# zprihoda/zopt

Hardware: AMD Instinct MI355X
Metric: LQR horizon-steps/sec (batch x T) at n=12,m=4,T=50 (higher is better)
Workload: dtype f64; 1 GPU; discreteFiniteHorizonLqr: 4096 random LTI systems per GPU, n=12 m=4 T=50 fp64, A/B/Q/R materialised (b,T,.,.), BASELINE configs[1]; batch_per_gpu=4096, T=50, n=12, m=4, parallelism=batch-sharded x1

## Files before the change

### zopt_amd/csrc/ilqr_backward.hip

```cpp
#include "dma_ring.h"
#include "models.h"
#include "ns16.h"
#include "tile16_f64.h"
#include "zm_common.h"

#include <cstdlib>

namespace zm {

template <int KS>
struct IlqrStepRegs {
    double F[KS];
    double C[KS];
    double Cu;
    double cv;
    double dc;
    double dr[KS];
};

struct TrajList {
    const int* list;
    long count;
};

template <int KS>
struct IlqrAddr {
    const double* pF0;
    const double* pC0;
    const double* pCu;
    const double* pcv;
    const double* pdc;
    const double* pdr0;
    const double* pz[4];
    int sz[4], stz[4];
    int zc[4];
    bool zlive[4];
    double* pOut;
    int dF, dC, sF, sC, sCu, scv, sOut, sd;
    bool rowok[KS], vF[KS], vC[KS], vCu, vcv, vOut, vL, cA;
    double vsum = 0.0;
    double cu_pad;
};

template <int KS, int MODE>
__device__ __forceinline__ void ilqr_load_step(IlqrStepRegs<KS>& d, IlqrAddr<KS>& a) {
    double f[KS], cc[KS];
#pragma unroll
    for (int s = 0; s < KS; ++s) f[s] = a.pF0[a.rowok[s] ? s * a.dF : 0];
    a.pF0 -= a.sF;
#pragma unroll
    for (int s = 0; s < KS; ++s) cc[s] = a.pC0[a.rowok[s] ? s * a.dC : 0];
    a.pC0 -= a.sC;
    const double cu = *a.pCu;
    a.pCu -= a.sCu;
    const double cv = *a.pcv;
    a.pcv -= a.scv;
#pragma unroll
    for (int s = 0; s < KS; ++s) {
        d.F[s] = a.vF[s] ? f[s] : 0.0;
        d.C[s] = a.vC[s] ? cc[s] : 0.0;
    }
    d.Cu = a.vCu ? cu : a.cu_pad;
    d.cv = a.vcv ? cv : 0.0;
    if constexpr (MODE == 1) {
        const double dc = *a.pdc;
        double dr[KS];
#pragma unroll
        for (int s = 0; s < KS; ++s) dr[s] = a.pdr0[a.rowok[s] ? 4 * s : 0];
        a.pdc -= a.sd;
        a.pdr0 -= a.sd;
        d.dc = a.cA ? dc : 0.0;
#pragma unroll
        for (int s = 0; s < KS; ++s) d.dr[s] = a.rowok[s] ? dr[s] : 0.0;
    }
}

constexpr int ILQR_LDS_DOUBLES = 116;

#ifdef ZM_SWEEP_LAB
__device__ unsigned long long zm_sweep_stamps[10];
struct SweepLab {
    unsigned long long acc[8], last;
};
#define ZM_SWEEP_STAMP(lab, q)                                                                         \
    do {                                                                                              \
        unsigned long long t_;                                                                        \
        asm volatile("s_memtime %0\n\ts_waitcnt lgkmcnt(0)" : "=s"(t_)::"memory");                    \
        (lab)->acc[q] += t_ - (lab)->last;                                                            \
        (lab)->last = t_;                                                                             \
    } while (0)
#else
struct SweepLab {};
#define ZM_SWEEP_STAMP(lab, q) do { } while (0)
#endif

__device__ __forceinline__ void ilqr_lds_sync() { wave_lds_sync(); }

template <int KS, int MODE, bool PREFETCH, bool ZIN = false>
__device__ __forceinline__ void ilqr_step(double (&Vxx)[KS], double (&vxr)[KS], IlqrStepRegs<KS>& d, IlqrAddr<KS>& a,
                                          double* sm, const int g, const int c, const int ob0, const int ob1,
                                          const int ob2, const int ob3, const int oqa, double* jA, const int n,
                                          const int m, const d4 zin = d4{0.0, 0.0, 0.0, 0.0}, SweepLab* lab = nullptr) {
    constexpr int NP = 4 * KS;
    d4 pz = zero4();
    if constexpr (MODE == 2 && ZIN) {
        d4 zt = zin;
        psd_project_ns<KS + 1, true>(zt, a.zlive, 1e-3, jA, g, c);
        pz = zt;
    } else if constexpr (MODE == 2) {
        double z[4] = {0.0, 0.0, 0.0, 0.0};
#pragma unroll
        for (int i0 = 0; i0 < NP; i0 += 4) {
            double fz[4][4];
#pragma unroll
            for (int i = 0; i < 4; ++i) {
                const int ic = (i0 + i) < n ? (i0 + i) : 0;
#pragma unroll
                for (int r = 0; r < 4; ++r) fz[i][r] = a.pz[r][(long)ic * a.sz[r]];
            }
#pragma unroll
            for (int i = 0; i < 4; ++i) {
                const double vxi = (i0 + i) < n ? sm[80 + i0 + i] : 0.0;
#pragma unroll
                for (int r = 0; r < 4; ++r) z[r] = __builtin_fma(vxi, fz[i][r], z[r]);
            }
        }
        d4 zt;
#pragma unroll
        for (int r = 0; r < 4; ++r) {
            a.pz[r] -= a.stz[r];
            zt[r] = (a.zc[r] >= 0) ? z[r] : 0.0;
        }
        psd_project_ns<KS + 1>(zt, a.zlive, 1e-3, jA, g, c);
        pz = zt;
    }
    d4 y = zero4();
#pragma unroll
    for (int s = 0; s < KS; ++s) y = mfma(Vxx[s], d.F[s], y);
    d4 gacc = zero4();
#pragma unroll
    for (int s = 0; s < KS; ++s) gacc[s] = d.C[s] + pz[s];
    gacc[KS] = d.Cu + pz[KS];
#pragma unroll
    for (int s = 0; s < KS; ++s) gacc = mfma(y[s], d.F[s], gacc);
    double qp = 0.0;
    if constexpr (MODE == 1) {
        double vtd = 0.0;
#pragma unroll
        for (int s = 0; s < KS; ++s) vtd = __builtin_fma(Vxx[s], d.dr[s], vtd);
        vtd = sum_xor16(vtd);
        vtd = sum_xor32(vtd);
        if (g == 0) sm[96 + c] = a.cA ? vtd : 0.0;
        ilqr_lds_sync();
#pragma unroll
        for (int s = 0; s < KS; ++s) {
            double vd = Vxx[s] * d.dc;
            vd = row16_sum(vd);
            const double w = vxr[s] + (a.cA ? vd : sm[96 + 4 * s + g]);
            qp = __builtin_fma(d.F[s], w, qp);
        }
    } else {
#pragma unroll
        for (int s = 0; s < KS; ++s) qp = __builtin_fma(d.F[s], vxr[s], qp);
    }
    qp = sum_xor16(qp);
    qp = sum_xor32(qp);
    const double qv = d.cv + qp;
    if constexpr (PREFETCH) ilqr_load_step<KS, MODE>(d, a);

    ZM_SWEEP_STAMP(lab, 2);
    sm[g * 16 + c] = gacc[KS];
    if (g == 0) sm[64 + c] = qv;
    __builtin_amdgcn_fence(__ATOMIC_RELEASE, "wavefront");
    __builtin_amdgcn_wave_barrier();
    __builtin_amdgcn_fence(__ATOMIC_ACQUIRE, "wavefront");
    double S[4][4], b[4], x[4];
#pragma unroll
    for (int i = 0; i < 4; ++i) {
#pragma unroll
        for (int jj = 0; jj < 4; ++jj) S[i][jj] = sm[i * 16 + NP + jj];
    }
    b[0] = sm[ob0];
    b[1] = sm[ob1];
    b[2] = sm[ob2];
    b[3] = sm[ob3];
    const double quu_a = sm[oqa];
    __builtin_amdgcn_wave_barrier();
    const double b0[4] = {b[0], b[1], b[2], b[3]};
    ZM_SWEEP_STAMP(lab, 3);
    if (__builtin_amdgcn_ballot_w64(!lu_solve4_nopivot(S, b, x)) != 0ull) lu_solve4_fallback(S, b, x);
    {
        double keep = x[0] + x[1] + x[2] + x[3];
        asm volatile("" : "+v"(keep));
    }
    ZM_SWEEP_STAMP(lab, 4);
    const double x01 = (g & 1) ? x[1] : x[0];
    const double x23 = (g & 1) ? x[3] : x[2];
    const double xg = (g & 2) ? x23 : x01;
    const double out = (MODE == 1) ? xg : -xg;
    if (a.vOut) *a.pOut = out;
    a.pOut -= a.sOut;
    const double lv = a.vL ? out : 0.0;
    double qu[4];
    if constexpr (MODE != 1) {
#pragma unroll
        for (int i = 0; i < 4; ++i) qu[i] = sm[64 + NP + i];
    }
    if constexpr (MODE != 1) {
        if (c == NP) a.vsum -= 0.5 * ((x[0] * qu[0] + x[1] * qu[1]) + (x[2] * qu[2] + x[3] * qu[3]));
    }

    double vxn = qv;
    if constexpr (MODE == 1) {
        if (g == 0 && c == NP) {
#pragma unroll
            for (int i = 0; i < 4; ++i) sm[112 + i] = x[i];
        }
        ilqr_lds_sync();
#pragma unroll
        for (int i = 0; i < 4; ++i) vxn = __builtin_fma(-b0[i], sm[112 + i], vxn);
    } else {
#pragma unroll
        for (int i = 0; i < 4; ++i) vxn = __builtin_fma(-x[i], qu[i], vxn);
    }
    if (g == 0) sm[80 + c] = a.cA ? vxn : 0.0;
    const d4 t1 = mfma(quu_a, lv, zero4());
    d4 vacc = zero4();
#pragma unroll
    for (int s = 0; s < KS; ++s) vacc[s] = gacc[s];
    vacc = mfma<true>(lv, t1[0], vacc);
#pragma unroll
    for (int s = 0; s < KS; ++s) Vxx[s] = vacc[s];
    ilqr_lds_sync();
#pragma unroll
    for (int s = 0; s < KS; ++s) vxr[s] = sm[80 + 4 * s + g];
    __builtin_amdgcn_wave_barrier();
    ZM_SWEEP_STAMP(lab, 5);
}

template <int KS, int MODE>
__global__ __launch_bounds__(64, 2) void ilqr_backward_t16_f64(
    const double* __restrict__ f_x, const double* __restrict__ f_u, const double* __restrict__ c_x,
    const double* __restrict__ c_u, const double* __restrict__ c_xx, const double* __restrict__ c_ux,
    const double* __restrict__ c_uu, const double* __restrict__ vf_x, const double* __restrict__ vf_xx,
    const double* __restrict__ dvec, const double* __restrict__ f_xx, const double* __restrict__ f_ux,
    const double* __restrict__ f_uu, const long svx, const long svxx, const int* __restrict__ active,
    const int shared_h, double* __restrict__ lout, double* __restrict__ Lout, const int T, const int n, const int m,
    const double* __restrict__ c_s, const double* __restrict__ vf_s, double* __restrict__ v_out,
    double* __restrict__ vx_out, double* __restrict__ vxx_out, const TrajList tl, const double* __restrict__ Hpk,
    const PairTab ptab) {
    constexpr int NP = 4 * KS;
    const int lane = threadIdx.x;
    const long traj = tl.list ? (long)tl.list[blockIdx.x] : (long)blockIdx.x;
    if (active && active[traj] == 0) return;
    const int g = lane >> 4, c = lane & 15;
    __shared__ double sm[ILQR_LDS_DOUBLES];
    __shared__ double jA[MODE == 2 ? NS_LDS_DOUBLES : 1];

    IlqrAddr<KS> a;
    const int nn = n * n, nm = n * m, mm = m * m;
    const bool cA = c < n;
    a.cA = cA;
    const bool cB = (c >= NP) && (c < NP + m);
    const long last = traj * T + (T - 1);
    const double* fxt = f_x + last * nn;
    const double* fut = f_u + last * nm;
    const double* cxt = c_x + last * n;
    const double* cut = c_u + last * m;
    const double* cxxt = shared_h ? c_xx : c_xx + last * nn;
    const double* cuxt = shared_h ? c_ux : c_ux + last * nm;
    const double* cuut = shared_h ? c_uu : c_uu + last * mm;
    a.sC = shared_h ? 0 : nn;
    const bool row0 = g < n;
    const bool laneA = row0 && cA, laneB = row0 && cB;
    a.dF = laneA ? 4 * n : laneB ? 4 * m : 0;
    a.sF = laneB ? nm : nn;
    a.dC = laneA ? 4 * n : 0;
#pragma unroll
    for (int s = 0; s < KS; ++s) {
        const int row = 4 * s + g;
        a.rowok[s] = row < n;
        a.vF[s] = (row < n) && (cA || cB);
        a.vC[s] = (row < n) && cA;
    }
    a.pF0 = laneA ? (fxt + g * n + c) : laneB ? (fut + g * m + (c - NP)) : fxt;
    a.pC0 = laneA ? (cxxt + g * n + c) : cxxt;
    const bool vux = (g < m) && cA, vuu = (g < m) && cB;
    a.vCu = vux || vuu;
    a.pCu = vux ? (cuxt + g * n + c) : vuu ? (cuut + g * m + (c - NP)) : cuxt;
    a.sCu = shared_h ? 0 : (vuu ? mm : nm);
    a.cu_pad = (g >= m && c == NP + g) ? 1.0 : 0.0;
    a.vcv = cA || cB;
    a.pcv = cA ? (cxt + c) : cB ? (cut + (c - NP)) : cxt;
    a.scv = cB ? m : n;
    if constexpr (MODE == 1) {
        const double* dt_ = dvec + last * n;
        a.pdc = cA ? (dt_ + c) : dt_;
        a.pdr0 = row0 ? (dt_ + g) : dt_;
        a.sd = n;
    }
    if constexpr (MODE == 2) {
        const long nnn = (long)nn * n, nmn = (long)nm * n, nmm = (long)nm * m;
        const double* fxxt = f_xx + last * nnn;
        const double* fuxt = f_ux + last * nmn;
        const double* fuut = f_uu + last * nmm;
#pragma unroll
        for (int r = 0; r < 4; ++r) {
            const int row = 4 * r + g;
            const bool rx = row < n, ru = (row >= NP) && (row < NP + m);
            const int ca = rx ? row : (ru ? n + (row - NP) : -1);
            const int cb = cA ? c : (cB ? n + (c - NP) : -1);
            a.zc[r] = (ca >= 0 && cb >= 0) ? ca * 17 + cb : -1;
            a.zlive[r] = (ca >= 0) && (row == c);
            if (Hpk != nullptr) {
                int pidx = -1;
                if (ca >= 0 && cb >= 0) {
                    const int lo = ca < cb ? ca : cb, hi = ca < cb ? cb : ca;
                    for (int q = 0; q < ptab.n; ++q) pidx = (ptab.ab[q] == (unsigned char)(lo * 16 + hi)) ? q : pidx;
                }
                const double* Hl = Hpk + last * (long)ptab.n * n;
                if (pidx >= 0) {
                    a.pz[r] = Hl + (long)pidx * n;  a.sz[r] = 1;  a.stz[r] = ptab.n * n;
                } else {
                    a.pz[r] = Hl;  a.sz[r] = 0;  a.stz[r] = ptab.n * n;
                    a.zc[r] = -1;
                }
            } else if (f_ux == nullptr && !(rx && cA)) {
                a.zc[r] = -1;
                a.pz[r] = fxxt;  a.sz[r] = 0;  a.stz[r] = (int)nnn;
            } else if (rx && cA) {
                a.pz[r] = fxxt + row * n + c;  a.sz[r] = nn;  a.stz[r] = (int)nnn;
            } else if (rx && cB) {
                a.pz[r] = fuxt + (c - NP) * n + row;  a.sz[r] = nm;  a.stz[r] = (int)nmn;
            } else if (ru && cA) {
                a.pz[r] = fuxt + (row - NP) * n + c;  a.sz[r] = nm;  a.stz[r] = (int)nmn;
            } else if (ru && cB) {
                a.pz[r] = fuut + (row - NP) * m + (c - NP);  a.sz[r] = mm;  a.stz[r] = (int)nmm;
            } else {
                a.pz[r] = fxxt;  a.sz[r] = 0;  a.stz[r] = (int)nnn;
            }
        }
    }
    a.vL = (g < m) && cA;
    const bool vl = (g < m) && (c == NP);
    a.vOut = a.vL || vl;
    a.pOut = a.vL ? (Lout + last * nm + g * n + c) : (lout + last * m + g);
    a.sOut = vl ? m : nm;

    const bool rhs_qu = (c == NP);
    const int ob0 = rhs_qu ? (64 + NP + 0) : (0 * 16 + c);
    const int ob1 = rhs_qu ? (64 + NP + 1) : (1 * 16 + c);
    const int ob2 = rhs_qu ? (64 + NP + 2) : (2 * 16 + c);
    const int ob3 = rhs_qu ? (64 + NP + 3) : (3 * 16 + c);
    const int oqa = (c < 4) ? (c * 16 + NP + g) : (g * 16 + c);

    double Vxx[KS], vxr[KS];
    {
        const double* vxx = shared_h ? vf_xx : vf_xx + traj * svxx;
        const double* vx = vf_x + traj * svx;
#pragma unroll
        for (int s = 0; s < KS; ++s) {
            const int row = 4 * s + g;
            const bool ok = (row < n) && cA;
            const double t = vxx[ok ? row * n + c : 0];
            Vxx[s] = ok ? t : 0.0;
            const double u = vx[row < n ? row : 0];
            vxr[s] = (row < n) ? u : 0.0;
        }
    }

    if (g == 0) sm[80 + c] = cA ? (vf_x + traj * svx)[c] : 0.0;
    ilqr_lds_sync();
    if constexpr (MODE == 2) {
        for (int k2 = T - 1; k2 >= 0; --k2) {
            IlqrStepRegs<KS> d;
            ilqr_load_step<KS, MODE>(d, a);
            ilqr_step<KS, MODE, false>(Vxx, vxr, d, a, sm, g, c, ob0, ob1, ob2, ob3, oqa, jA, n, m);
        }
    } else {
    IlqrStepRegs<KS> d0, d1;
    ilqr_load_step<KS, MODE>(d0, a);
    if (T >= 2) ilqr_load_step<KS, MODE>(d1, a);
    int k = T - 1;
    while (k >= 3) {
        ilqr_step<KS, MODE, true>(Vxx, vxr, d0, a, sm, g, c, ob0, ob1, ob2, ob3, oqa, jA, n, m);
        ilqr_step<KS, MODE, true>(Vxx, vxr, d1, a, sm, g, c, ob0, ob1, ob2, ob3, oqa, jA, n, m);
        k -= 2;
    }
    if (k == 2) {
        ilqr_step<KS, MODE, true>(Vxx, vxr, d0, a, sm, g, c, ob0, ob1, ob2, ob3, oqa, jA, n, m);
        ilqr_step<KS, MODE, false>(Vxx, vxr, d1, a, sm, g, c, ob0, ob1, ob2, ob3, oqa, jA, n, m);
        ilqr_step<KS, MODE, false>(Vxx, vxr, d0, a, sm, g, c, ob0, ob1, ob2, ob3, oqa, jA, n, m);
    } else if (k == 1) {
        ilqr_step<KS, MODE, false>(Vxx, vxr, d0, a, sm, g, c, ob0, ob1, ob2, ob3, oqa, jA, n, m);
        ilqr_step<KS, MODE, false>(Vxx, vxr, d1, a, sm, g, c, ob0, ob1, ob2, ob3, oqa, jA, n, m);
    } else {
        ilqr_step<KS, MODE, false>(Vxx, vxr, d0, a, sm, g, c, ob0, ob1, ob2, ob3, oqa, jA, n, m);
    }
    }
    if (vxx_out) {
#pragma unroll
        for (int s = 0; s < KS; ++s) {
            const int row = 4 * s + g;
            if (row < n && cA) vxx_out[traj * nn + row * n + c] = Vxx[s];
        }
    }
    if (vx_out && g == 0 && cA) vx_out[traj * n + c] = sm[80 + c];
    if (v_out) {
        double cs = 0.0;
        if (c_s)
            for (int k2 = lane; k2 < T; k2 += 64) cs += c_s[traj * T + k2];
#pragma unroll
        for (int off = 32; off >= 1; off >>= 1) cs += __shfl_xor(cs, off, 64);
        if (g == 0 && c == NP) v_out[traj] = ((vf_s ? vf_s[traj] : 0.0) + cs) + a.vsum;
    }
}

}


namespace zm {

struct JacTab {
    unsigned char pos[12 * 16];
};
struct HTab {
    unsigned short dense[96];
    int n;
};
template <int N, int M, bool SHARED, int MODE, int NPAIR = 0, int NJP = 0, int NHS = 0>
struct IlqrDmaGeom {
    static constexpr int KS = N / 4;
    static constexpr int CFX = NJP ? NJP / 2 : N * N / 2, CFU = NJP ? 0 : N * M / 2, CCX = N / 2, CCU = M / 2;
    static constexpr int CXX = SHARED ? 0 : N * N / 2, CUX = SHARED ? 0 : N * M / 2, CUU = SHARED ? 0 : M * M / 2;
    static constexpr int CD = (MODE == 1) ? N / 2 : 0;
    static constexpr int CH = (MODE == 2) ? (NHS ? NHS / 2 : NPAIR * N / 2) : 0;
    static constexpr int CT = CFX + CFU + CCX + CCU + CXX + CUX + CUU + CD + CH;
    static constexpr int NI = (CT + 63) / 64;
    static constexpr int SLOT = NI * 1024;
    static constexpr int OFX = 0, OFU = CFX * 16, OCX = OFU + CFU * 16, OCU = OCX + CCX * 16;
    static constexpr int OXX = OCU + CCU * 16, OUX = OXX + CXX * 16, OUU = OUX + CUX * 16;
    static constexpr int OD = OUU + CUU * 16;
    static constexpr int OH = OD + CD * 16;
    static constexpr int OZ = CT * 16;
    static constexpr int OONE = OZ + 16;
    static_assert(NJP % 2 == 0 && (NJP == 0 || (N == 12 && SHARED)), "packed Jacobians: n = 12, 16-B rows, shared cost Hessians");
    static_assert(NJP == 0 || SLOT - OZ >= 32, "slot needs a zero and a one chunk");
    static_assert(N % 4 == 0 && N >= 8 && N <= 12 && M == 4, "fast path: all K-step rows live, m = 4");
    static_assert(MODE == 0 || (MODE == 1 && !SHARED) || (MODE == 2 && SHARED && N == 12 && NPAIR > 0 && NPAIR <= ZM_MAX_PAIRS),
                  "iLQR, affine LQR, or DDP with shared cost Hessians and packed second derivatives");
    static_assert(SLOT - OZ >= 16, "slot needs zero padding");
};

constexpr int ILQR_DMA_WAVES = 3, DDP_DMA_WAVES = 2;
template <int N, int M, int D, bool SHARED, int MODE, int NPAIR = 0, int NJP = 0, int NHS = 0, int W = 1>
__global__ __launch_bounds__(64 * W, MODE == 2 ? DDP_DMA_WAVES : ILQR_DMA_WAVES) void ilqr_backward_dma_f64(
    const double* __restrict__ f_x, const double* __restrict__ f_u, const double* __restrict__ c_x,
    const double* __restrict__ c_u, const double* __restrict__ c_xx, const double* __restrict__ c_ux,
    const double* __restrict__ c_uu, const double* __restrict__ vf_x, const double* __restrict__ vf_xx,
    const double* __restrict__ dvec, const long svx, const long svxx, const int* __restrict__ active,
    double* __restrict__ lout, double* __restrict__ Lout, const int T, const TrajList tl, const double* __restrict__ Hpk,
    const PairTab ptab, const JacTab jtab, const HTab htab) {
    using G = IlqrDmaGeom<N, M, SHARED, MODE, NPAIR, NJP, NHS>;
    static_assert(NHS % 2 == 0 && NHS <= 96 && (NHS == 0 || MODE == 2), "sparse second derivatives: DDP mode, 16-B rows");
    constexpr int KS = G::KS, NI = G::NI, SLOT = G::SLOT, NP = N;
    constexpr int nn = N * N, nm = N * M, mm = M * M;
    constexpr int SMO = D * SLOT;
    constexpr int HDN = NHS ? NPAIR * N : 0;
    constexpr int PER_WAVE = SMO + ILQR_LDS_DOUBLES * 8 + (MODE == 2 ? NS_LDS_DOUBLES * 8 : 0) + HDN * 8;
    static_assert(PER_WAVE % 16 == 0, "per-wave LDS slices stay 16-B aligned");
    __shared__ __attribute__((aligned(16))) char lds_all[W * PER_WAVE];
    const int wave = (W == 1) ? 0 : __builtin_amdgcn_readfirstlane((int)(threadIdx.x >> 6));
    char* const lds = lds_all + wave * PER_WAVE;
    double* sm = (double*)(lds + SMO);
    double* jA = (double*)(lds + SMO + ILQR_LDS_DOUBLES * 8);
    double* hd = jA + NS_LDS_DOUBLES;
    const int lane = threadIdx.x & 63;
    const long slot_ = (long)blockIdx.x * W + wave;
    if (W > 1 && slot_ >= tl.count) return;
    const long traj = tl.list ? (long)tl.list[slot_] : slot_;
    if (active && active[traj] == 0) return;
    const int g = lane >> 4, c = lane & 15;
    const bool cA = c < N, cB = (c >= N) && (c < N + M);

    const char* p[NI];
    int st[NI];
    {
        const long last = traj * T + (T - 1);
#pragma unroll
        for (int i = 0; i < NI; ++i) {
            int q = i * 64 + lane;
            const char* src = (NJP && q == G::CT + 1) ? (const char*)zm_one_src : (const char*)zm_zero_src;
            int stride = 0;
            if (q < G::CFX) {
                if constexpr (NJP != 0) {
                    src = (const char*)(f_x + last * NJP) + q * 16;  stride = NJP * 8;
                } else {
                    src = (const char*)(f_x + last * nn) + q * 16;  stride = nn * 8;
                }
            } else if ((q -= G::CFX) < G::CFU) {
                src = (const char*)(f_u + last * nm) + q * 16;  stride = nm * 8;
            } else if ((q -= G::CFU) < G::CCX) {
                src = (const char*)(c_x + last * N) + q * 16;   stride = N * 8;
            } else if ((q -= G::CCX) < G::CCU) {
                src = (const char*)(c_u + last * M) + q * 16;   stride = M * 8;
            } else if constexpr (MODE == 2) {
                if ((q -= G::CCU) < G::CH) {
                    constexpr int HROW = NHS ? NHS : NPAIR * N;
                    src = (const char*)(Hpk + last * (long)HROW) + q * 16;  stride = HROW * 8;
                }
            } else if constexpr (!SHARED) {
                if ((q -= G::CCU) < G::CXX) {
                    src = (const char*)(c_xx + last * nn) + q * 16;  stride = nn * 8;
                } else if ((q -= G::CXX) < G::CUX) {
                    src = (const char*)(c_ux + last * nm) + q * 16;  stride = nm * 8;
                } else if ((q -= G::CUX) < G::CUU) {
                    src = (const char*)(c_uu + last * mm) + q * 16;  stride = mm * 8;
                } else if constexpr (MODE == 1) {
                    if ((q -= G::CUU) < G::CD) {
                        src = (const char*)(dvec + last * N) + q * 16;  stride = N * 8;
                    }
                }
            }
            p[i] = src;
            st[i] = stride;
        }
    }
    auto dma = [&](char* slot) {
#pragma unroll
        for (int i = 0; i < NI; ++i) {
            __builtin_amdgcn_global_load_lds((glb_void_t*)p[i], (lds_void_t*)(slot + i * 1024), 16, 0, 0);
            p[i] -= st[i];
        }
    };
    const int oF = cA ? (G::OFX + (g * N + c) * 8) : cB ? (G::OFU + (g * M + (c - N)) * 8) : G::OZ;
    const int dF = cA ? 4 * N * 8 : cB ? 4 * M * 8 : 0;
    int oFp[KS];
#pragma unroll
    for (int s = 0; s < KS; ++s) {
        const int row = 4 * s + g;
        const int p = NJP ? (int)jtab.pos[row * 16 + c] : 255;
        oFp[s] = (p != 255) ? (G::OFX + p * 8) : ((row == c) ? G::OONE : G::OZ);
    }
    const int ocv = cA ? (G::OCX + c * 8) : cB ? (G::OCU + (c - N) * 8) : G::OZ;
    const int oC = cA ? (G::OXX + (g * N + c) * 8) : G::OZ;
    const int dC = cA ? 4 * N * 8 : 0;
    const int oCu = cA ? (G::OUX + (g * N + c) * 8) : cB ? (G::OUU + (g * M + (c - N)) * 8) : G::OZ;
    const int odc = cA ? (G::OD + c * 8) : G::OZ;

    IlqrAddr<KS> a;
    a.cA = cA;
    a.vL = cA;
    const bool vl = (c == NP);
    a.vOut = a.vL || vl;
    {
        const long last = traj * T + (T - 1);
        a.pOut = a.vL ? (Lout + last * nm + g * N + c) : (lout + last * M + g);
    }
    a.sOut = vl ? M : nm;
    int oH[4];
    bool zok[4];
    if constexpr (MODE == 2) {
#pragma unroll
        for (int r = 0; r < 4; ++r) {
            const int row = 4 * r + g;
            const int lo = row < c ? row : c, hi = row < c ? c : row;
            int pidx = -1;
            for (int q = 0; q < NPAIR; ++q) pidx = (ptab.ab[q] == (unsigned char)(lo * 16 + hi)) ? q : pidx;
            zok[r] = pidx >= 0;
            oH[r] = (NHS ? 0 : G::OH) + (pidx >= 0 ? pidx : 0) * (N * 8);
            a.zlive[r] = (row == c);
        }
    }
    const bool rhs_qu = (c == NP);
    const int ob0 = rhs_qu ? (64 + NP + 0) : (0 * 16 + c);
    const int ob1 = rhs_qu ? (64 + NP + 1) : (1 * 16 + c);
    const int ob2 = rhs_qu ? (64 + NP + 2) : (2 * 16 + c);
    const int ob3 = rhs_qu ? (64 + NP + 3) : (3 * 16 + c);
    const int oqa = (c < 4) ? (c * 16 + NP + g) : (g * 16 + c);

    double Csh[KS], Cush = 0.0;
#pragma unroll
    for (int s = 0; s < KS; ++s) Csh[s] = 0.0;
    if constexpr (SHARED) {
#pragma unroll
        for (int s = 0; s < KS; ++s) {
            const double t = c_xx[cA ? (4 * s + g) * N + c : 0];
            Csh[s] = cA ? t : 0.0;
        }
        const double tu = cA ? c_ux[g * N + c] : (cB ? c_uu[g * M + (c - N)] : 0.0);
        Cush = tu;
    }
    double Vxx[KS], vxr[KS];
    {
        const double* vxx = SHARED ? vf_xx : vf_xx + traj * svxx;
        const double* vx = vf_x + traj * svx;
#pragma unroll
        for (int s = 0; s < KS; ++s) {
            const int row = 4 * s + g;
            const double t = vxx[cA ? row * N + c : 0];
            Vxx[s] = cA ? t : 0.0;
            vxr[s] = vx[row];
        }
        if (g == 0) sm[80 + c] = cA ? vx[c] : 0.0;
    }
    int hdst0 = 0, hdst1 = 0;
    if constexpr (NHS != 0) {
        for (int e = lane; e < HDN; e += 64) hd[e] = 0.0;
        hdst0 = (lane < htab.n) ? (int)htab.dense[lane] : -1;
        hdst1 = (lane + 64 < htab.n) ? (int)htab.dense[(lane + 64) % 96] : -1;
    }
    ilqr_lds_sync();

#pragma unroll
    for (int i = 0; i < D; ++i)
        if (T - 1 - i >= 0) dma(lds + i * SLOT);
    int j = T - 1;
#ifdef ZM_SWEEP_LAB
    SweepLab labv;
    for (int q = 0; q < 8; ++q) labv.acc[q] = 0ull;
    asm volatile("s_memtime %0\n\ts_waitcnt lgkmcnt(0)" : "=s"(labv.last)::"memory");
    SweepLab* const lab = &labv;
#else
    SweepLab* const lab = nullptr;
#endif
    for (;;) {
#pragma unroll
        for (int si = 0; si < D; ++si) {
            char* slot = lds + si * SLOT;
            wait_for_step<NI, D>(j);
            ZM_SWEEP_STAMP(lab, 0);
            IlqrStepRegs<KS> d;
#pragma unroll
            for (int s = 0; s < KS; ++s) d.F[s] = *(const double*)(slot + (NJP ? oFp[s] : oF + s * dF));
            d.cv = *(const double*)(slot + ocv);
            if constexpr (SHARED) {
#pragma unroll
                for (int s = 0; s < KS; ++s) d.C[s] = Csh[s];
                d.Cu = Cush;
            } else {
#pragma unroll
                for (int s = 0; s < KS; ++s) d.C[s] = *(const double*)(slot + oC + s * dC);
                d.Cu = *(const double*)(slot + oCu);
            }
            if constexpr (MODE == 1) {
                d.dc = *(const double*)(slot + odc);
#pragma unroll
                for (int s = 0; s < KS; ++s) d.dr[s] = *(const double*)(slot + G::OD + (4 * s + g) * 8);
            }
            d4 zin = zero4();
            if constexpr (NHS != 0) {
                const double* hs = (const double*)(slot + G::OH);
                const double h0 = hs[lane], h1 = hs[(lane + 64 < NHS) ? lane + 64 : 0];
                if (hdst0 >= 0) hd[hdst0] = h0;
                if (hdst1 >= 0) hd[hdst1] = h1;
                ilqr_lds_sync();
            }
            if constexpr (MODE == 2) {
                double vx[N];
#pragma unroll
                for (int i = 0; i < N; ++i) vx[i] = sm[80 + i];
#pragma unroll
                for (int r = 0; r < 4; ++r) {
                    const double* h = NHS ? (const double*)((const char*)hd + oH[r]) : (const double*)(slot + oH[r]);
                    double z = 0.0;
#pragma unroll
                    for (int i = 0; i < N; ++i) z = __builtin_fma(vx[i], h[i], z);
                    zin[r] = zok[r] ? z : 0.0;
                }
            }
            asm volatile("s_waitcnt lgkmcnt(0)" ::: "memory");
            if (j - D >= 0) dma(slot);
            ZM_SWEEP_STAMP(lab, 1);
            ilqr_step<KS, MODE, false, MODE == 2>(Vxx, vxr, d, a, sm, g, c, ob0, ob1, ob2, ob3, oqa, jA, N, M, zin, lab);
            if (--j < 0) {
#ifdef ZM_SWEEP_LAB
                if (blockIdx.x == 0 && threadIdx.x == 0) {
                    for (int q = 0; q < 8; ++q) atomicAdd(&zm_sweep_stamps[q], labv.acc[q]);
                    atomicAdd(&zm_sweep_stamps[8], 1ull);
                }
#endif
                return;
            }
        }
    }
}

template <int MODE>
static int ilqr_backward_dma_dispatch(const double* f_x, const double* f_u, const double* c_x, const double* c_u,
                                      const double* c_xx, const double* c_ux, const double* c_uu, const double* vf_x,
                                      const double* vf_xx, const double* dvec, long svx, long svxx, const int* act, int sh,
                                      double* l, double* L, int64_t batch, int T, int n, int m, hipStream_t st,
                                      TrajList tl = TrajList{nullptr, 0}) {
    static const bool off = [] {
        const char* e = zm::fallback_env("ZOPT_AMD_ILQR_PATH");
        return e && e[0] == 'r';
    }();
    if (off || m != 4 || (n != 8 && n != 12)) return ZM_EUNSUPPORTED;
    const uintptr_t al = (uintptr_t)f_x | (uintptr_t)f_u | (uintptr_t)c_x | (uintptr_t)c_u | (uintptr_t)dvec |
                         (sh ? 0 : ((uintptr_t)c_xx | (uintptr_t)c_ux | (uintptr_t)c_uu));
    if (al & 15) return ZM_EUNSUPPORTED;
    const dim3 grid((unsigned)(tl.list ? tl.count : batch)), block(64);
    constexpr int DS = 3, DF = 2;
#define ZM_LAUNCH_ILQR_DMA(NN, DD, SH)                                                                                     \
    hipLaunchKernelGGL((ilqr_backward_dma_f64<NN, 4, DD, SH, MODE>), grid, block, 0, st, f_x, f_u, c_x, c_u, c_xx, c_ux, c_uu, \
                       vf_x, vf_xx, dvec, svx, svxx, act, l, L, T, tl, (const double*)nullptr, PairTab{}, JacTab{}, HTab{})
    if constexpr (MODE == 0) {
        if (n == 12) {
            if (sh) ZM_LAUNCH_ILQR_DMA(12, DS, true); else ZM_LAUNCH_ILQR_DMA(12, DF, false);
        } else {
            if (sh) ZM_LAUNCH_ILQR_DMA(8, DS, true); else ZM_LAUNCH_ILQR_DMA(8, DF, false);
        }
    } else {
        if (n == 12) ZM_LAUNCH_ILQR_DMA(12, DF, false); else ZM_LAUNCH_ILQR_DMA(8, DF, false);
    }
#undef ZM_LAUNCH_ILQR_DMA
    ZM_HIP_CHECK(hipGetLastError());
    return ZM_OK;
}

static int ddp_backward_dma_dispatch(const double* f_x, const double* f_u, const double* Hpk, const PairTab& ptab, const double* c_x,
                                     const double* c_u, const double* c_xx, const double* c_ux, const double* c_uu, const double* vf_x,
                                     const double* vf_xx, long svx, const int* act, int sh, double* l, double* L, int64_t batch, int T,
                                     int n, int m, hipStream_t st, TrajList tl) {
    static const bool off = [] {
        const char* e = zm::fallback_env("ZOPT_AMD_ILQR_PATH");
        return e && e[0] == 'r';
    }();
    if (off || !sh || n != 12 || m != 4 || ptab.n != 28 || !Hpk) return ZM_EUNSUPPORTED;
    if (((uintptr_t)f_x | (uintptr_t)f_u | (uintptr_t)c_x | (uintptr_t)c_u | (uintptr_t)Hpk) & 15) return ZM_EUNSUPPORTED;
    const dim3 grid((unsigned)(tl.list ? tl.count : batch)), block(64);
    hipLaunchKernelGGL((ilqr_backward_dma_f64<12, 4, 2, true, 2, 28>), grid, block, 0, st, f_x, f_u, c_x, c_u, c_xx, c_ux, c_uu, vf_x,
                       vf_xx, (const double*)nullptr, svx, 0L, act, l, L, T, tl, Hpk, ptab, JacTab{}, HTab{});
    ZM_HIP_CHECK(hipGetLastError());
    return ZM_OK;
}

int sweep_packed_jacobians(const double* Fp, int njp, const unsigned char* pos, const double* Hpk, const PairTab& ptab, const double* c_x,
                           const double* c_u, const double* c_xx, const double* c_ux, const double* c_uu, const double* vf_x,
                           const double* vf_xx, const int* act, double* l, double* L, int64_t batch, int T, hipStream_t st, TrajList tl,
                           int nhs, const unsigned short* hdense, int nh) {
    if (((uintptr_t)Fp | (uintptr_t)c_x | (uintptr_t)c_u | (uintptr_t)Hpk) & 15) return ZM_EUNSUPPORTED;
    if ((njp != 56 && njp != 60) || (Hpk && ptab.n != 28)) return ZM_EUNSUPPORTED;
    if (nhs && !(Hpk && ((njp == 56 && nhs == 70) || (njp == 60 && nhs == 86)) && hdense && nh > 0 && nh <= nhs)) return ZM_EUNSUPPORTED;
    JacTab jt;
    for (int e = 0; e < 192; ++e) jt.pos[e] = pos[e];
    HTab ht{};
    for (int e = 0; e < nh && nhs; ++e) ht.dense[e] = hdense[e];
    ht.n = nhs ? nh : 0;
    const long nslot = tl.list ? tl.count : batch;
    static const long wg4_max = [] {
        const char* e = zm::lab_env("ZOPT_AMD_SWEEP_WG4");
        return e ? atol(e) : 2048L;
    }();
    const bool quad_wg = tl.list && nslot <= wg4_max;
    const dim3 grid((unsigned)(quad_wg ? (nslot + 3) / 4 : nslot)), block(quad_wg ? 256 : 64);
#define ZM_LAUNCH_PACKED(DD, MODE_, NPAIR_, NJP_, NHS_)                                                                               \
    do {                                                                                                                              \
        if (quad_wg)                                                                                                                  \
            hipLaunchKernelGGL((ilqr_backward_dma_f64<12, 4, DD, true, MODE_, NPAIR_, NJP_, NHS_, 4>), grid, block, 0, st, Fp,         \
                               (const double*)nullptr, c_x, c_u, c_xx, c_ux, c_uu, vf_x, vf_xx, (const double*)nullptr, 12L, 0L, act, l, \
                               L, T, tl, Hpk, ptab, jt, ht);                                                                          \
        else                                                                                                                          \
            hipLaunchKernelGGL((ilqr_backward_dma_f64<12, 4, DD, true, MODE_, NPAIR_, NJP_, NHS_>), grid, block, 0, st, Fp,            \
                               (const double*)nullptr, c_x, c_u, c_xx, c_ux, c_uu, vf_x, vf_xx, (const double*)nullptr, 12L, 0L, act, l, \
                               L, T, tl, Hpk, ptab, jt, ht);                                                                          \
    } while (0)
    if (Hpk && nhs) {
        if (njp == 56) ZM_LAUNCH_PACKED(2, 2, 28, 56, 70); else ZM_LAUNCH_PACKED(2, 2, 28, 60, 86);
    } else if (Hpk) {
        if (njp == 56) ZM_LAUNCH_PACKED(2, 2, 28, 56, 0); else ZM_LAUNCH_PACKED(2, 2, 28, 60, 0);
    } else {
        if (njp == 56) ZM_LAUNCH_PACKED(3, 0, 0, 56, 0); else ZM_LAUNCH_PACKED(3, 0, 0, 60, 0);
    }
#undef ZM_LAUNCH_PACKED
    ZM_HIP_CHECK(hipGetLastError());
    return ZM_OK;
}

}

namespace zm {
struct DdpTensors {
    const double *f_xx, *f_ux, *f_uu;
    const double* Hpk = nullptr;
    PairTab ptab = PairTab{};
};
struct ValueIO {
    const double *c, *vf;
    double *v_out, *vx_out, *vxx_out;
};

template <int MODE>
static int launch_ilqr(const double* f_x, const double* f_u, const double* c_x, const double* c_u, const double* c_xx,
                       const double* c_ux, const double* c_uu, const double* vf_x, const double* vf_xx, const double* d,
                       long svx, long svxx, const int* act, int sh, double* l, double* L, int64_t batch, int T, int n, int m,
                       hipStream_t st, DdpTensors z = DdpTensors{nullptr, nullptr, nullptr},
                       ValueIO v = ValueIO{nullptr, nullptr, nullptr, nullptr, nullptr}, TrajList tl = TrajList{nullptr, 0}) {
    const dim3 grid((unsigned)(tl.list ? tl.count : batch)), block(64);
    if (n <= 4)
        hipLaunchKernelGGL((ilqr_backward_t16_f64<1, MODE>), grid, block, 0, st, f_x, f_u, c_x, c_u, c_xx, c_ux, c_uu, vf_x,
                           vf_xx, d, z.f_xx, z.f_ux, z.f_uu, svx, svxx, act, sh, l, L, T, n, m, v.c, v.vf, v.v_out, v.vx_out, v.vxx_out, tl, z.Hpk, z.ptab);
    else if (n <= 8)
        hipLaunchKernelGGL((ilqr_backward_t16_f64<2, MODE>), grid, block, 0, st, f_x, f_u, c_x, c_u, c_xx, c_ux, c_uu, vf_x,
                           vf_xx, d, z.f_xx, z.f_ux, z.f_uu, svx, svxx, act, sh, l, L, T, n, m, v.c, v.vf, v.v_out, v.vx_out, v.vxx_out, tl, z.Hpk, z.ptab);
    else
        hipLaunchKernelGGL((ilqr_backward_t16_f64<3, MODE>), grid, block, 0, st, f_x, f_u, c_x, c_u, c_xx, c_ux, c_uu, vf_x,
                           vf_xx, d, z.f_xx, z.f_ux, z.f_uu, svx, svxx, act, sh, l, L, T, n, m, v.c, v.vf, v.v_out, v.vx_out, v.vxx_out, tl, z.Hpk, z.ptab);
    ZM_HIP_CHECK(hipGetLastError());
    return ZM_OK;
}
}

namespace zm {
int sweep_tiled_f64_dispatch(int mode, const double* f_x, const double* f_u, const double* c_x, const double* c_u, const double* c_xx,
                             const double* c_ux, const double* c_uu, const double* vf_x, const double* vf_xx, const double* dvec,
                             long svx, long svxx, const int* active, int shared_hessian, double* l, double* L, int64_t batch, int T,
                             int n, int m, hipStream_t st, const int* list, long count, const double* cs = nullptr,
                             const double* vf = nullptr, double* v_out = nullptr, double* vx_out = nullptr, double* vxx_out = nullptr);
}

static int zm_check_sweep_args(const char* who, int64_t batch, int T, int n, int m, bool tiled = false) {
    if (batch < 0 || T < 1 || n < 1 || m < 1)
        return zm::set_error(ZM_EINVAL, "%s: bad size batch=%lld T=%d n=%d m=%d", who, (long long)batch, T, n, m);
    if (tiled ? (n > 48 || m > 16) : (n > 12 || m > 4))
        return zm::set_error(ZM_EUNSUPPORTED, "%s: (n=%d, m=%d) not covered (need %s)", who, n, m,
                             tiled ? "n<=48, m<=16" : "n<=12, m<=4");
    if ((int64_t)T * n * n >= (int64_t)1 << 31 || batch >= ((int64_t)1 << 31))
        return zm::set_error(ZM_EUNSUPPORTED, "%s: T*n*n or batch too large", who);
    return ZM_OK;
}

extern "C" int zm_ilqr_backward_list_f64(const double* f_x, const double* f_u, const double* c_x, const double* c_u,
                                         const double* c_xx, const double* c_ux, const double* c_uu, const double* vf_x,
                                         const double* vf_xx, const int32_t* list, int64_t count, const int32_t* active,
                                         int shared_hessian, double* l, double* L, int64_t batch, int T, int n, int m,
                                         void* stream) {
    if (batch == 0 || (list && count == 0)) return ZM_OK;
    if (list && (count < 0 || count > batch)) return zm::set_error(ZM_EINVAL, "zm_ilqr_backward_list_f64: bad list length");
    const zm::TrajList tl{(const int*)list, (long)count};
    if (!f_x || !f_u || !c_x || !c_u || !c_xx || !c_ux || !c_uu || !vf_x || !vf_xx || !l || !L)
        return zm::set_error(ZM_EINVAL, "zm_ilqr_backward_f64: null pointer");
    const int rc = zm_check_sweep_args("zm_ilqr_backward_f64", batch, T, n, m, true);
    if (rc) return rc;
    if (n > 12 || m > 4)
        return zm::sweep_tiled_f64_dispatch(0, f_x, f_u, c_x, c_u, c_xx, c_ux, c_uu, vf_x, vf_xx, nullptr, (long)n, (long)n * n,
                                            (const int*)active, shared_hessian ? 1 : 0, l, L, batch, T, n, m, (hipStream_t)stream,
                                            (const int*)list, (long)count);
    if (zm::ilqr_backward_dma_dispatch<0>(f_x, f_u, c_x, c_u, c_xx, c_ux, c_uu, vf_x, vf_xx, nullptr, (long)n, (long)n * n,
                                       (const int*)active, shared_hessian ? 1 : 0, l, L, batch, T, n, m,
                                       (hipStream_t)stream, tl) == ZM_OK)
        return ZM_OK;
    return zm::launch_ilqr<0>(f_x, f_u, c_x, c_u, c_xx, c_ux, c_uu, vf_x, vf_xx, nullptr, (long)n, (long)n * n,
                              (const int*)active, shared_hessian ? 1 : 0, l, L, batch, T, n, m, (hipStream_t)stream,
                              zm::DdpTensors{nullptr, nullptr, nullptr}, zm::ValueIO{nullptr, nullptr, nullptr, nullptr, nullptr}, tl);
}

extern "C" int zm_ilqr_backward_ex_f64(const double* f_x, const double* f_u, const double* c_x, const double* c_u,
                                       const double* c_xx, const double* c_ux, const double* c_uu, const double* vf_x,
                                       const double* vf_xx, const int32_t* active, int shared_hessian, double* l,
                                       double* L, int64_t batch, int T, int n, int m, void* stream) {
    return zm_ilqr_backward_list_f64(f_x, f_u, c_x, c_u, c_xx, c_ux, c_uu, vf_x, vf_xx, nullptr, 0, active, shared_hessian, l, L,
                                     batch, T, n, m, stream);
}

extern "C" int zm_ilqr_backward_f64(const double* f_x, const double* f_u, const double* c_x, const double* c_u,
                                    const double* c_xx, const double* c_ux, const double* c_uu, const double* vf_x,
                                    const double* vf_xx, double* l, double* L, int64_t batch, int T, int n, int m,
                                    void* stream) {
    if (batch == 0) return ZM_OK;
    return zm_ilqr_backward_ex_f64(f_x, f_u, c_x, c_u, c_xx, c_ux, c_uu, vf_x, vf_xx, nullptr, 0, l, L, batch, T, n, m,
                                   stream);
}

extern "C" int zm_lqr_backward_affine_f64(const double* A, const double* B, const double* d, const double* Q,
                                          const double* R, const double* H, const double* q, const double* r, double* L,
                                          double* l, int64_t batch, int T, int n, int m, void* stream) {
    if (batch == 0) return ZM_OK;
    if (!A || !B || !d || !Q || !R || !H || !q || !r || !L || !l)
        return zm::set_error(ZM_EINVAL, "zm_lqr_backward_affine_f64: null pointer");
    const int rc = zm_check_sweep_args("zm_lqr_backward_affine_f64", batch, T, n, m, true);
    if (rc) return rc;
    if (batch == 0) return ZM_OK;
    const double* vf_xx = Q + (int64_t)(T - 1) * n * n;
    const double* vf_x = q + (int64_t)(T - 1) * n;
    if (n > 12 || m > 4)
        return zm::sweep_tiled_f64_dispatch(1, A, B, q, r, Q, H, R, vf_x, vf_xx, d, (long)T * n, (long)T * n * n, nullptr, 0, l, L, batch,
                                            T, n, m, (hipStream_t)stream, nullptr, 0);
    if (zm::ilqr_backward_dma_dispatch<1>(A, B, q, r, Q, H, R, vf_x, vf_xx, d, (long)T * n, (long)T * n * n, nullptr, 0, l, L,
                                          batch, T, n, m, (hipStream_t)stream) == ZM_OK)
        return ZM_OK;
    return zm::launch_ilqr<1>(A, B, q, r, Q, H, R, vf_x, vf_xx, d, (long)T * n, (long)T * n * n, nullptr, 0, l, L, batch, T,
                              n, m, (hipStream_t)stream);
}

extern "C" int zm_ddp_backward_list_f64(const double* f_x, const double* f_u, const double* f_xx, const double* f_ux,
                                        const double* f_uu, const double* c_x, const double* c_u, const double* c_xx,
                                        const double* c_ux, const double* c_uu, const double* vf_x, const double* vf_xx,
                                        const int32_t* list, int64_t count, const int32_t* active, int shared_hessian,
                                        double* l, double* L, int64_t batch, int T, int n, int m, void* stream) {
    if (batch == 0 || (list && count == 0)) return ZM_OK;
    if (list && (count < 0 || count > batch)) return zm::set_error(ZM_EINVAL, "zm_ddp_backward_list_f64: bad list length");
    if (!f_x || !f_u || !f_xx || (!f_ux != !f_uu) || !c_x || !c_u || !c_xx || !c_ux || !c_uu || !vf_x || !vf_xx || !l || !L)
        return zm::set_error(ZM_EINVAL, "zm_ddp_backward_f64: null pointer (f_ux and f_uu may be NULL together: identically zero)");
    const int rc = zm_check_sweep_args("zm_ddp_backward_f64", batch, T, n, m);
    if (rc) return rc;
    if ((int64_t)n * n * n >= (int64_t)1 << 31) return zm::set_error(ZM_EUNSUPPORTED, "zm_ddp_backward_f64: n too large");
    if (batch == 0) return ZM_OK;
    return zm::launch_ilqr<2>(f_x, f_u, c_x, c_u, c_xx, c_ux, c_uu, vf_x, vf_xx, nullptr, (long)n, (long)n * n,
                              (const int*)active, shared_hessian ? 1 : 0, l, L, batch, T, n, m, (hipStream_t)stream,
                              zm::DdpTensors{f_xx, f_ux, f_uu}, zm::ValueIO{nullptr, nullptr, nullptr, nullptr, nullptr},
                              zm::TrajList{(const int*)list, (long)count});
}

extern "C" int zm_ddp_backward_pairs_list_f64(const zm_model_t* model, const double* f_x, const double* f_u, const double* H,
                                              const double* c_x, const double* c_u, const double* c_xx, const double* c_ux,
                                              const double* c_uu, const double* vf_x, const double* vf_xx, const int32_t* list,
                                              int64_t count, const int32_t* active, int shared_hessian, double* l, double* L,
                                              int64_t batch, int T, void* stream) {
    if (batch == 0 || (list && count == 0)) return ZM_OK;
    if (list && (count < 0 || count > batch)) return zm::set_error(ZM_EINVAL, "zm_ddp_backward_pairs_list_f64: bad list length");
    if (!model || !f_x || !f_u || !H || !c_x || !c_u || !c_xx || !c_ux || !c_uu || !vf_x || !vf_xx || !l || !L)
        return zm::set_error(ZM_EINVAL, "zm_ddp_backward_pairs_list_f64: null pointer");
    const int n = model->n, m = model->m;
    const int rc = zm_check_sweep_args("zm_ddp_backward_pairs_list_f64", batch, T, n, m);
    if (rc) return rc;
    const zm::PairTab pt = zm::model_pair_table(model->kind);
    if (pt.n < 1)
        return zm::set_error(ZM_EUNSUPPORTED, "zm_ddp_backward_pairs_list_f64: the model declares no Hessian pairs");
    const zm::TrajList tl{(const int*)list, (long)count};
    {
        const int rd = zm::ddp_backward_dma_dispatch(f_x, f_u, H, pt, c_x, c_u, c_xx, c_ux, c_uu, vf_x, vf_xx, (long)n, (const int*)active,
                                                     shared_hessian ? 1 : 0, l, L, batch, T, n, m, (hipStream_t)stream, tl);
        if (rd != ZM_EUNSUPPORTED) return rd;
    }
    zm::DdpTensors z{nullptr, nullptr, nullptr, H, pt};
    return zm::launch_ilqr<2>(f_x, f_u, c_x, c_u, c_xx, c_ux, c_uu, vf_x, vf_xx, nullptr, (long)n, (long)n * n, (const int*)active,
                              shared_hessian ? 1 : 0, l, L, batch, T, n, m, (hipStream_t)stream, z,
                              zm::ValueIO{nullptr, nullptr, nullptr, nullptr, nullptr}, tl);
}

extern "C" int zm_ddp_backward_f64(const double* f_x, const double* f_u, const double* f_xx, const double* f_ux,
                                   const double* f_uu, const double* c_x, const double* c_u, const double* c_xx,
                                   const double* c_ux, const double* c_uu, const double* vf_x, const double* vf_xx,
                                   const int32_t* active, int shared_hessian, double* l, double* L, int64_t batch, int T,
                                   int n, int m, void* stream) {
    return zm_ddp_backward_list_f64(f_x, f_u, f_xx, f_ux, f_uu, c_x, c_u, c_xx, c_ux, c_uu, vf_x, vf_xx, nullptr, 0, active,
                                    shared_hessian, l, L, batch, T, n, m, stream);
}

extern "C" int zm_riccati_value_f64(const double* f_x, const double* f_u, const double* f_xx, const double* f_ux,
                                    const double* f_uu, const double* c, const double* c_x, const double* c_u,
                                    const double* c_xx, const double* c_ux, const double* c_uu, const double* vf,
                                    const double* vf_x, const double* vf_xx, double* l, double* L, double* v_out,
                                    double* vx_out, double* vxx_out, int64_t batch, int T, int n, int m, void* stream) {
    if (batch == 0) return ZM_OK;
    if (!f_x || !f_u || !c_x || !c_u || !c_xx || !c_ux || !c_uu || !vf_x || !vf_xx || !l || !L)
        return zm::set_error(ZM_EINVAL, "zm_riccati_value_f64: null pointer");
    const bool ddp = f_xx || f_ux || f_uu;
    if (ddp && (!f_xx || (!f_ux != !f_uu)))
        return zm::set_error(ZM_EINVAL, "zm_riccati_value_f64: f_xx goes with f_ux and f_uu (the latter two may be NULL together: zero)");
    const int rc = zm_check_sweep_args("zm_riccati_value_f64", batch, T, n, m, !ddp);
    if (rc) return rc;
    if (!ddp && (n > 12 || m > 4)) {
        if (!v_out || !vx_out || !vxx_out) return zm::set_error(ZM_EINVAL, "zm_riccati_value_f64: the value outputs are required at n > 12 or m > 4");
        return zm::sweep_tiled_f64_dispatch(0, f_x, f_u, c_x, c_u, c_xx, c_ux, c_uu, vf_x, vf_xx, nullptr, (long)n, (long)n * n, nullptr, 0,
                                            l, L, batch, T, n, m, (hipStream_t)stream, nullptr, 0, c, vf, v_out, vx_out, vxx_out);
    }
    const zm::ValueIO v{c, vf, v_out, vx_out, vxx_out};
    if (ddp)
        return zm::launch_ilqr<2>(f_x, f_u, c_x, c_u, c_xx, c_ux, c_uu, vf_x, vf_xx, nullptr, (long)n, (long)n * n, nullptr, 0, l,
                                  L, batch, T, n, m, (hipStream_t)stream, zm::DdpTensors{f_xx, f_ux, f_uu}, v);
    return zm::launch_ilqr<0>(f_x, f_u, c_x, c_u, c_xx, c_ux, c_uu, vf_x, vf_xx, nullptr, (long)n, (long)n * n, nullptr, 0, l, L,
                              batch, T, n, m, (hipStream_t)stream, zm::DdpTensors{nullptr, nullptr, nullptr}, v);
}

#ifdef ZM_SWEEP_LAB
extern "C" int zm_lab_sweep_stamps(unsigned long long* out, int reset) {
    ZM_HIP_CHECK(hipDeviceSynchronize());
    ZM_HIP_CHECK(hipMemcpyFromSymbol(out, HIP_SYMBOL(zm::zm_sweep_stamps), sizeof(unsigned long long) * 10));
    if (reset) {
        unsigned long long z[10] = {0};
        ZM_HIP_CHECK(hipMemcpyToSymbol(HIP_SYMBOL(zm::zm_sweep_stamps), z, sizeof(z)));
    }
    return ZM_OK;
}
#endif
```

Before: 1.640 billion horizon-steps/s.

## Replace per-lane 4x4 LU solve with distributed cofactor-adjugate solve via MFMA

Replaces the per-lane 4x4 LU solve of Quu x = b, where each lane reloaded the full 16-element matrix and RHS from LDS, with a distributed adjugate method. Each lane loads a 3x3 minor, computes one cofactor, and then uses 4x4x4 f64 MFMAs to form adj*b and the determinant, which is scaled by a fast reciprocal. The value-function updates (vxn and the vsum reduction) are also rewritten as MFMA and cross-lane reductions, removing an extra LDS round trip. A fallback to the pivoted LU runs when the determinant check or an identity check fails, at the cost of extra checks and possible precision loss for ill-conditioned Quu.

```diff
diff --git a/zopt_amd/csrc/ilqr_backward.hip b/zopt_amd/csrc/ilqr_backward.hip
--- a/zopt_amd/csrc/ilqr_backward.hip
+++ b/zopt_amd/csrc/ilqr_backward.hip
@@ -1,6 +1,7 @@
 #include "dma_ring.h"
 #include "models.h"
 #include "ns16.h"
+#include "solve4_cofactor.h"
 #include "tile16_f64.h"
 #include "zm_common.h"
 
@@ -98,9 +99,9 @@
 
 template <int KS, int MODE, bool PREFETCH, bool ZIN = false>
 __device__ __forceinline__ void ilqr_step(double (&Vxx)[KS], double (&vxr)[KS], IlqrStepRegs<KS>& d, IlqrAddr<KS>& a,
-                                          double* sm, const int g, const int c, const int ob0, const int ob1,
-                                          const int ob2, const int ob3, const int oqa, double* jA, const int n,
-                                          const int m, const d4 zin = d4{0.0, 0.0, 0.0, 0.0}, SweepLab* lab = nullptr) {
+                                          double* sm, const int g, const int c, const Cof4Lane<MODE == 2>& cl,
+                                          const int oqa, double* jA, const int n, const int m,
+                                          const d4 zin = d4{0.0, 0.0, 0.0, 0.0}, SweepLab* lab = nullptr) {
     constexpr int NP = 4 * KS;
     d4 pz = zero4();
     if constexpr (MODE == 2 && ZIN) {
@@ -169,59 +170,40 @@
     if constexpr (PREFETCH) ilqr_load_step<KS, MODE>(d, a);
 
     ZM_SWEEP_STAMP(lab, 2);
-    sm[g * 16 + c] = gacc[KS];
+    const double srow = gacc[KS];
+    sm[g * 16 + c] = srow;
     if (g == 0) sm[64 + c] = qv;
-    __builtin_amdgcn_fence(__ATOMIC_RELEASE, "wavefront");
-    __builtin_amdgcn_wave_barrier();
-    __builtin_amdgcn_fence(__ATOMIC_ACQUIRE, "wavefront");
-    double S[4][4], b[4], x[4];
-#pragma unroll
-    for (int i = 0; i < 4; ++i) {
-#pragma unroll
-        for (int jj = 0; jj < 4; ++jj) S[i][jj] = sm[i * 16 + NP + jj];
-    }
-    b[0] = sm[ob0];
-    b[1] = sm[ob1];
-    b[2] = sm[ob2];
-    b[3] = sm[ob3];
-    const double quu_a = sm[oqa];
-    __builtin_amdgcn_wave_barrier();
-    const double b0[4] = {b[0], b[1], b[2], b[3]};
+    ilqr_lds_sync();
+    double qg = sm[64 + NP + g];
+    double quu_a = 0.0;
+    if constexpr (MODE != 2) quu_a = sm[oqa];
     ZM_SWEEP_STAMP(lab, 3);
-    if (__builtin_amdgcn_ballot_w64(!lu_solve4_nopivot(S, b, x)) != 0ull) lu_solve4_fallback(S, b, x);
-    {
-        double keep = x[0] + x[1] + x[2] + x[3];
-        asm volatile("" : "+v"(keep));
-    }
+    double xs, xl;
+    solve4_cofactor<NP>(sm, cl, srow, qg, g, c, xs, xl);
+#ifdef ZM_SWEEP_LAB
+    asm volatile("" : "+v"(xs), "+v"(xl));
+#endif
     ZM_SWEEP_STAMP(lab, 4);
-    const double x01 = (g & 1) ? x[1] : x[0];
-    const double x23 = (g & 1) ? x[3] : x[2];
-    const double xg = (g & 2) ? x23 : x01;
+    if constexpr (MODE == 2) {
+        wave_lds_sync();
+        qg = sm[64 + NP + g];
+        quu_a = sm[oqa];
+    }
+    const double xg = (c == NP) ? xl : xs;
     const double out = (MODE == 1) ? xg : -xg;
     if (a.vOut) *a.pOut = out;
     a.pOut -= a.sOut;
     const double lv = a.vL ? out : 0.0;
-    double qu[4];
     if constexpr (MODE != 1) {
-#pragma unroll
-        for (int i = 0; i < 4; ++i) qu[i] = sm[64 + NP + i];
-    }
-    if constexpr (MODE != 1) {
-        if (c == NP) a.vsum -= 0.5 * ((x[0] * qu[0] + x[1] * qu[1]) + (x[2] * qu[2] + x[3] * qu[3]));
-    }
-
-    double vxn = qv;
+        const double xq = sum_xor32(sum_xor16(xl * qg));
+        if (c == NP) a.vsum -= 0.5 * xq;
+    }
+
+    double vxn;
     if constexpr (MODE == 1) {
-        if (g == 0 && c == NP) {
-#pragma unroll
-            for (int i = 0; i < 4; ++i) sm[112 + i] = x[i];
-        }
-        ilqr_lds_sync();
-#pragma unroll
-        for (int i = 0; i < 4; ++i) vxn = __builtin_fma(-b0[i], sm[112 + i], vxn);
+        vxn = __builtin_amdgcn_mfma_f64_4x4x4f64(-xl, srow, qv, 0, 0, 0);
     } else {
-#pragma unroll
-        for (int i = 0; i < 4; ++i) vxn = __builtin_fma(-x[i], qu[i], vxn);
+        vxn = __builtin_amdgcn_mfma_f64_4x4x4f64(-qg, xs, qv, 0, 0, 0);
     }
     if (g == 0) sm[80 + c] = a.cA ? vxn : 0.0;
     const d4 t1 = mfma(quu_a, lv, zero4());
@@ -347,11 +329,7 @@
     a.pOut = a.vL ? (Lout + last * nm + g * n + c) : (lout + last * m + g);
     a.sOut = vl ? m : nm;
 
-    const bool rhs_qu = (c == NP);
-    const int ob0 = rhs_qu ? (64 + NP + 0) : (0 * 16 + c);
-    const int ob1 = rhs_qu ? (64 + NP + 1) : (1 * 16 + c);
-    const int ob2 = rhs_qu ? (64 + NP + 2) : (2 * 16 + c);
-    const int ob3 = rhs_qu ? (64 + NP + 3) : (3 * 16 + c);
+    const Cof4Lane<MODE == 2> cl = cof4_lane<NP, MODE == 2>(g, c);
     const int oqa = (c < 4) ? (c * 16 + NP + g) : (g * 16 + c);
 
     double Vxx[KS], vxr[KS];
@@ -375,7 +353,7 @@
         for (int k2 = T - 1; k2 >= 0; --k2) {
             IlqrStepRegs<KS> d;
             ilqr_load_step<KS, MODE>(d, a);
-            ilqr_step<KS, MODE, false>(Vxx, vxr, d, a, sm, g, c, ob0, ob1, ob2, ob3, oqa, jA, n, m);
+            ilqr_step<KS, MODE, false>(Vxx, vxr, d, a, sm, g, c, cl, oqa, jA, n, m);
         }
     } else {
     IlqrStepRegs<KS> d0, d1;
@@ -383,19 +361,19 @@
     if (T >= 2) ilqr_load_step<KS, MODE>(d1, a);
     int k = T - 1;
     while (k >= 3) {
-        ilqr_step<KS, MODE, true>(Vxx, vxr, d0, a, sm, g, c, ob0, ob1, ob2, ob3, oqa, jA, n, m);
-        ilqr_step<KS, MODE, true>(Vxx, vxr, d1, a, sm, g, c, ob0, ob1, ob2, ob3, oqa, jA, n, m);
+        ilqr_step<KS, MODE, true>(Vxx, vxr, d0, a, sm, g, c, cl, oqa, jA, n, m);
+        ilqr_step<KS, MODE, true>(Vxx, vxr, d1, a, sm, g, c, cl, oqa, jA, n, m);
         k -= 2;
     }
     if (k == 2) {
-        ilqr_step<KS, MODE, true>(Vxx, vxr, d0, a, sm, g, c, ob0, ob1, ob2, ob3, oqa, jA, n, m);
-        ilqr_step<KS, MODE, false>(Vxx, vxr, d1, a, sm, g, c, ob0, ob1, ob2, ob3, oqa, jA, n, m);
-        ilqr_step<KS, MODE, false>(Vxx, vxr, d0, a, sm, g, c, ob0, ob1, ob2, ob3, oqa, jA, n, m);
+        ilqr_step<KS, MODE, true>(Vxx, vxr, d0, a, sm, g, c, cl, oqa, jA, n, m);
+        ilqr_step<KS, MODE, false>(Vxx, vxr, d1, a, sm, g, c, cl, oqa, jA, n, m);
+        ilqr_step<KS, MODE, false>(Vxx, vxr, d0, a, sm, g, c, cl, oqa, jA, n, m);
     } else if (k == 1) {
-        ilqr_step<KS, MODE, false>(Vxx, vxr, d0, a, sm, g, c, ob0, ob1, ob2, ob3, oqa, jA, n, m);
-        ilqr_step<KS, MODE, false>(Vxx, vxr, d1, a, sm, g, c, ob0, ob1, ob2, ob3, oqa, jA, n, m);
+        ilqr_step<KS, MODE, false>(Vxx, vxr, d0, a, sm, g, c, cl, oqa, jA, n, m);
+        ilqr_step<KS, MODE, false>(Vxx, vxr, d1, a, sm, g, c, cl, oqa, jA, n, m);
     } else {
-        ilqr_step<KS, MODE, false>(Vxx, vxr, d0, a, sm, g, c, ob0, ob1, ob2, ob3, oqa, jA, n, m);
+        ilqr_step<KS, MODE, false>(Vxx, vxr, d0, a, sm, g, c, cl, oqa, jA, n, m);
     }
     }
     if (vxx_out) {
@@ -572,11 +550,7 @@
             a.zlive[r] = (row == c);
         }
     }
-    const bool rhs_qu = (c == NP);
-    const int ob0 = rhs_qu ? (64 + NP + 0) : (0 * 16 + c);
-    const int ob1 = rhs_qu ? (64 + NP + 1) : (1 * 16 + c);
-    const int ob2 = rhs_qu ? (64 + NP + 2) : (2 * 16 + c);
-    const int ob3 = rhs_qu ? (64 + NP + 3) : (3 * 16 + c);
+    const Cof4Lane<MODE == 2> cl = cof4_lane<NP, MODE == 2>(g, c);
     const int oqa = (c < 4) ? (c * 16 + NP + g) : (g * 16 + c);
 
     double Csh[KS], Cush = 0.0;
@@ -672,7 +646,7 @@
             asm volatile("s_waitcnt lgkmcnt(0)" ::: "memory");
             if (j - D >= 0) dma(slot);
             ZM_SWEEP_STAMP(lab, 1);
-            ilqr_step<KS, MODE, false, MODE == 2>(Vxx, vxr, d, a, sm, g, c, ob0, ob1, ob2, ob3, oqa, jA, N, M, zin, lab);
+            ilqr_step<KS, MODE, false, MODE == 2>(Vxx, vxr, d, a, sm, g, c, cl, oqa, jA, N, M, zin, lab);
             if (--j < 0) {
 #ifdef ZM_SWEEP_LAB
                 if (blockIdx.x == 0 && threadIdx.x == 0) {
diff --git a/zopt_amd/csrc/solve4_cofactor.h b/zopt_amd/csrc/solve4_cofactor.h
--- /dev/null
+++ b/zopt_amd/csrc/solve4_cofactor.h
@@ -0,0 +1,96 @@
+#pragma once
+#include "tile16_f64.h"
+#include "zm_common.h"
+
+namespace zm {
+
+template <bool COMPACT>
+struct Cof4Lane;
+template <>
+struct Cof4Lane<false> {
+    int mo[3][3];
+    double eye;
+    bool cS;
+};
+template <>
+struct Cof4Lane<true> {
+    unsigned pk;
+};
+
+template <int NP, bool COMPACT>
+__device__ __forceinline__ Cof4Lane<COMPACT> cof4_lane(const int g, const int c) {
+    const int cc = c & 3;
+    int mr[3] = {g == 0 ? 1 : 0, g <= 1 ? 2 : 1, g <= 2 ? 3 : 2};
+    const int mc[3] = {cc == 0 ? 1 : 0, cc <= 1 ? 2 : 1, cc <= 2 ? 3 : 2};
+    if ((g + cc) & 1) { const int t = mr[1]; mr[1] = mr[2]; mr[2] = t; }
+    Cof4Lane<COMPACT> L;
+    if constexpr (COMPACT) {
+        static_assert(3 * 16 + NP < 64, "row starts fit six bits");
+        L.pk = 0u;
+#pragma unroll
+        for (int k = 0; k < 3; ++k) L.pk |= (unsigned)(mr[k] * 16 + NP) << (6 * k) | (unsigned)mc[k] << (18 + 2 * k);
+    } else {
+#pragma unroll
+        for (int k = 0; k < 3; ++k)
+#pragma unroll
+            for (int l = 0; l < 3; ++l) L.mo[k][l] = mr[k] * 16 + NP + mc[l];
+        L.cS = (c >= NP) && (c < NP + 4);
+        L.eye = (L.cS && g == c - NP) ? 1.0 : 0.0;
+    }
+    return L;
+}
+
+template <int NP, bool COMPACT>
+__device__ __forceinline__ void solve4_cofactor(double* sm, const Cof4Lane<COMPACT>& L, const double srow, const double qg, const int g,
+                                                const int c, double& xs, double& xl) {
+    double mi[3][3];
+    bool cS;
+    double eye;
+    if constexpr (COMPACT) {
+        unsigned pk = L.pk;
+        asm volatile("" : "+v"(pk));
+#pragma unroll
+        for (int k = 0; k < 3; ++k)
+#pragma unroll
+            for (int l = 0; l < 3; ++l) mi[k][l] = sm[((pk >> (6 * k)) & 63u) + ((pk >> (18 + 2 * l)) & 3u)];
+        cS = (c >= NP) && (c < NP + 4);
+        eye = (cS && g == c - NP) ? 1.0 : 0.0;
+    } else {
+#pragma unroll
+        for (int k = 0; k < 3; ++k)
+#pragma unroll
+            for (int l = 0; l < 3; ++l) mi[k][l] = sm[L.mo[k][l]];
+        cS = L.cS;
+        eye = L.eye;
+    }
+    const double cof = cofactor3(mi);
+    const double X = __builtin_amdgcn_mfma_f64_4x4x4f64(cof, srow, 0.0, 0, 0, 0);
+    const double Xl = __builtin_amdgcn_mfma_f64_4x4x4f64(cof, qg, 0.0, 0, 0, 0);
+    const double det = readlane_f64(X, NP);
+    const double r = fast_rcp(det);
+    xs = X * r;
+    xl = Xl * r;
+    const bool ok = (__builtin_fabs(det) <= 1.79769313486231570815e308) & (__builtin_fabs(r) <= 1.79769313486231570815e308) &
+                    (!cS || __builtin_fabs(__builtin_fma(-eye, det, X)) <= 0x1p-45 * __builtin_fabs(det));
+    if (__builtin_amdgcn_ballot_w64(!ok) != 0ull) {
+        const bool ql = (c == NP);
+        double S[4][4], b[4], x[4];
+#pragma unroll
+        for (int i = 0; i < 4; ++i) {
+#pragma unroll
+            for (int jj = 0; jj < 4; ++jj) S[i][jj] = sm[i * 16 + NP + jj];
+            b[i] = sm[ql ? (64 + NP + i) : (i * 16 + c)];
+        }
+        lu_solve4_fallback(S, b, x);
+        const double x01 = (g & 1) ? x[1] : x[0];
+        const double x23 = (g & 1) ? x[3] : x[2];
+        xs = (g & 2) ? x23 : x01;
+        wave_lds_sync();
+        if (ql) sm[112 + g] = xs;
+        wave_lds_sync();
+        xl = sm[112 + g];
+        wave_lds_sync();
+    }
+}
+
+}
```

Result: no change. 1.644 billion horizon-steps/s (median of 2 runs) (+0.2%).
